# HDaoud/ORBSLAMM

Hardware: AMD Instinct MI355X
Metric: frames/s ORB extract+match, 1241x376 @2000 kp; bit-exact kp/desc vs CPU (higher is better)
Workload: dtype u8

## Files before the change

### include/orbslamm_hip.h

```cpp
#ifndef ORBSLAMM_HIP_H
#define ORBSLAMM_HIP_H

#include <stddef.h>
#include <stdint.h>

#ifdef __cplusplus
extern "C" {
#endif

#define ORBX_MAX_LEVELS 16

enum {
    ORBX_OK = 0,
    ORBX_E_INVALID = -1,
    ORBX_E_NO_DEVICE = -2,
    ORBX_E_HIP = -3,
    ORBX_E_CAPACITY = -4,
    ORBX_E_UNSUPPORTED = -5
};

const char* orbx_last_error(void);
int orbx_device_count(void);
int orbx_device_pci_bus_id(int device, char* out, int cap);
int orbx_device_shader_clock_mhz(int device, float* mhz);
// ... 101 lines not shown
    double ms[ORBX_PROF_MAX];
    int64_t launches[ORBX_PROF_MAX];
} OrbxProfile;
int orbx_set_serial(orbx_t* h, int serial);
int orbx_profile_enable(orbx_t* h, int enable);
int orbx_profile_select(orbx_t* h, const char* kernel);
int orbx_profile_read(orbx_t* h, OrbxProfile* out, int reset);

int orbx_debug_pair_overlap(orbx_t* h, int nb, float target_ms, int* n_kernels, const char** names,
                            float* alone_ms, float* co_ms, int32_t* lds_bytes, int32_t* wg_threads, int32_t* wgs);

int orbx_debug_link_rate(orbx_t* h, size_t up_bytes, size_t down_bytes, int reps, float* h2d_gbs, float* d2h_gbs,
                         float* both_up_gbs, float* both_down_gbs);

int orbx_debug_stage_rows(uint8_t* dst, size_t dpitch, const uint8_t* src, size_t spitch, size_t w, int rows);

typedef struct orbm_handle orbm_t;
int orbm_create(int device, orbm_t** out);
void orbm_destroy(orbm_t* h);
int orbm_thread_handle(int device, orbm_t** out);
int orbm_alloc_stats(orbm_t* h, int64_t* device_allocs, int64_t* host_allocs, int64_t* handles_made);

int orbm_distance_matrix(orbm_t* h, const uint8_t* q, int nq, const uint8_t* t, int nt, int32_t* dist);

int orbm_match_bruteforce(orbm_t* h, const uint8_t* qdesc, const float* qangle, int nq,
                          const uint8_t* tdesc, const float* tangle, int nt,
                          float nnratio, int th_low, int check_ori, int32_t* match, int* nmatches);

typedef struct {
    int32_t n_nodes;
// ... 321 lines not shown
```

### orbslamm_amd/_lib.py

```python
import ctypes as C
import os
import subprocess

import numpy as np

_PKG = os.path.dirname(os.path.abspath(__file__))
_ROOT = os.path.dirname(_PKG)
SO_PATH = os.path.join(_PKG, "liborbslamm_hip.so")
SRC = os.path.join(_PKG, "csrc", "orbslamm_hip.hip")
HIPCC_FLAGS = ["--offload-arch=gfx950", "-O3", "-std=c++17", "-ffp-contract=off", "-fPIC", "-shared"]

ORBX_MAX_LEVELS = 16
ORBX_PROF_MAX = 16
ORBX_OK, ORBX_E_INVALID, ORBX_E_NO_DEVICE, ORBX_E_HIP, ORBX_E_CAPACITY, ORBX_E_UNSUPPORTED = 0, -1, -2, -3, -4, -5

KP_DTYPE = np.dtype([("x", "<f4"), ("y", "<f4"), ("size", "<f4"), ("angle", "<f4"),
                     ("response", "<f4"), ("octave", "<i4"), ("class_id", "<i4")])
assert KP_DTYPE.itemsize == 28


class OrbxParams(C.Structure):
    _fields_ = [("nfeatures", C.c_int32), ("scaleFactor", C.c_float), ("nlevels", C.c_int32),
                ("iniThFAST", C.c_int32), ("minThFAST", C.c_int32)]

# ... 24 lines not shown
    _fields_ = [("minX", C.c_float), ("minY", C.c_float), ("invW", C.c_float), ("invH", C.c_float),
                ("cols", C.c_int32), ("rows", C.c_int32)]


class OrbmProjParams(C.Structure):
    _fields_ = [("mode", C.c_int32), ("nnratio", C.c_float), ("check_ori", C.c_int32), ("th_dist", C.c_int32)]


EXPORTS = [
    "orbx_last_error", "orbx_device_count", "orbx_device_pci_bus_id", "orbx_device_shader_clock_mhz", "orbx_create", "orbx_create_live", "orbx_destroy", "orbx_levels", "orbx_scale_factor",
    "orbx_scale_tables", "orbx_features_per_level", "orbx_umax", "orbx_max_keypoints", "orbx_extract",
    "orbx_extract_batch", "orbx_submit_batch", "orbx_submit_batch_into", "orbx_collect", "orbx_host_alloc", "orbx_collect_view", "orbx_release", "orbx_collect_batch", "orbx_extract_match_batch",
    "orbx_host_alloc_frames", "orbx_host_free", "orbx_host_register", "orbx_host_unregister", "orbx_extract_batch_device", "orbx_device_results", "orbx_download",
    "orbx_pyramid_level", "orbx_compute_stereo_matches", "orbx_level_candidates", "orbx_sync", "orbx_device_alloc", "orbx_device_free", "orbx_upload", "orbx_match_prev_batch_device",
    "orbx_device_matches", "orbx_download_matches", "orbx_reset_stream", "orbx_set_serial", "orbx_profile_enable",
    "orbx_profile_read", "orbx_debug_pair_overlap", "orbx_debug_link_rate", "orbx_debug_stage_rows", "orbx_profile_select", "orbm_create", "orbm_destroy", "orbm_thread_handle", "orbm_alloc_stats", "orbm_distance_matrix", "orbm_match_bruteforce",
    "orbm_search_by_bow", "orbm_search_by_projection", "orbm_search_by_projection_stereo", "orbm_projection_prepare", "orbm_features_in_area", "orbm_window_best",
    "orbm_search_for_initialization", "orbm_search_for_triangulation", "orbm_distinctive_descriptors", "orbm_descriptors_to_text", "orbm_descriptors_from_text", "orbm_undistort_keypoints", "orbm_compute_stereo_from_rgbd", "orbm_frame_create", "orbm_frame_destroy", "orbm_frame_size", "orbm_frame_settle",
    "orbm_frame_download_keys_un", "orbm_search_by_projection_frame", "orbm_frame_compute_bow", "orbm_search_by_bow_frames", "orbm_search_for_initialization_frames", "orbm_window_best_frame", "orbm_search_for_triangulation_frames",
    "orbv_create", "orbv_load_text", "orbv_destroy", "orbv_transform", "orbv_score",
    "orbm_last_search_stats", "orbm_frameset_create", "orbm_frameset_destroy", "orbm_frameset_build", "orbm_frameset_build_from_extractor",
    "orbm_frameset_sync", "orbm_frameset_attach", "orbm_frameset_download", "orbm_track_frames", "orbm_track_local_points", "orbm_track_frame_projected", "orbm_track_results", "orbm_track_stats",
    "orbm_frameset_compute_bow", "orbm_frameset_bow_vector", "orbm_bow_frames", "orbm_bow_results",
]

EXPORTS_KFDB = [
    "orbk_pool_create", "orbk_pool_destroy", "orbk_pool_size", "orbk_pool_set_bow", "orbk_pool_set_bow_from_frameset", "orbk_pool_score",
    "orbk_pool_set_covisibility", "orbk_pool_read_state", "orbk_db_create", "orbk_db_destroy", "orbk_db_add", "orbk_db_erase", "orbk_db_clear",
    "orbk_db_size", "orbk_db_empty", "orbk_db_last_scored", "orbk_detect_relocalization_candidates",
    "orbk_detect_relocalization_candidates_frameset", "orbk_detect_loop_candidates", "orbk_detect_loop_batch",
]
# ... 157 lines not shown
```

### orbslamm_amd/csrc/orbx_geometry.inc

```

static int init_tables(orbx_handle* h)
{
    const OrbxParams& p = h->prm;
    if (p.nlevels < 1 || p.nlevels > ORBX_MAXL || p.nfeatures < 1 || !(p.scaleFactor > 1.0f))
        return fail(ORBX_E_INVALID, "bad ORBextractor parameters");
    const int L = p.nlevels;
    h->nlevels = L;
    const double scaleFactor = (double)p.scaleFactor;
    h->mvScaleFactor[0] = 1.0f;
    h->mvLevelSigma2[0] = 1.0f;
    for (int i = 1; i < L; i++) {
        h->mvScaleFactor[i] = (float)((double)h->mvScaleFactor[i - 1] * scaleFactor);
        h->mvLevelSigma2[i] = h->mvScaleFactor[i] * h->mvScaleFactor[i];
    }
    for (int i = 0; i < L; i++) {
        h->mvInvScaleFactor[i] = 1.0f / h->mvScaleFactor[i];
        h->mvInvLevelSigma2[i] = 1.0f / h->mvLevelSigma2[i];
    }
    const float factor = (float)(1.0 / scaleFactor);
    float nDesired = (float)p.nfeatures * (1 - factor) / (1 - (float)pow((double)factor, (double)L));
    int sum = 0;
    for (int l = 0; l < L - 1; l++) {
        h->mnFeaturesPerLevel[l] = cv_round(nDesired);
        sum += h->mnFeaturesPerLevel[l];
// ... 10 lines not shown
    for (v = kHalfPatch, v0 = 0; v >= vmin; --v) {
        while (h->umax[v0] == h->umax[v0 + 1]) ++v0;
        h->umax[v] = v0;
        ++v0;
    }
    return ORBX_OK;
}

struct HostGeom {
    Geom g;
    std::vector<Cell> cells;
    std::vector<short4> tabs;
    int xoff[ORBX_MAXL], yoff[ORBX_MAXL];
    int tileStrideDw, tileRows, fastListCap, tileRows0, fastListCap0, fastSmapPitch, fastSmapPitch0, nodeCap;
    BlurTiles bt;
    KpBlocks kb;
    int kbTotal;
    std::vector<PyrRange> pyrRanges;
    int pyrBlocks, pyrBufA, pyrBufB, pyrTabCap;
    bool pyrFused;
};

static inline size_t pyr_lds_bytes(int bufA, int bufB, int tabCap) { return ((size_t)bufA + bufB) * 4 + (size_t)tabCap * 16; }

static int build_geometry(const orbx_handle* h, int w, int h0, HostGeom& out)
{
    Geom& g = out.g;
    memset(&g, 0, sizeof g);
    g.nlevels = h->nlevels;
    g.w0 = w; g.h0 = h0;
// ... 117 lines not shown
            auto sat = [](float v) { long r = lrintf(v); return (short)(r > 32767 ? 32767 : (r < -32768 ? -32768 : r)); };
            xt[dx] = make_short4((short)sx, sat((1.f - fx) * 2048), sat(fx * 2048), 0);
        }
        for (int dx = 0; dx < dw; dx++) xt[dx].w = dx < xmax ? 1 : 0;
        out.tabs.insert(out.tabs.end(), xt.begin(), xt.end());
        out.yoff[l] = (int)out.tabs.size();
        for (int dy = 0; dy < dh; dy++) {
            float fy = (float)((dy + 0.5) * scale_y - 0.5);
            int sy = (int)std::floor(fy);
            fy -= sy;
            auto clip = [&](int y) { return y < 0 ? 0 : (y < sh ? y : sh - 1); };
            auto sat = [](float v) { long r = lrintf(v); return (short)(r > 32767 ? 32767 : (r < -32768 ? -32768 : r)); };
            out.tabs.push_back(make_short4((short)clip(sy), (short)clip(sy + 1), sat((1.f - fy) * 2048), sat(fy * 2048)));
        }
    }
    int tb = 0, kb = 0;
    for (int l = 0; l < g.nlevels; l++) {
        out.bt.base[l] = tb;
        out.bt.tilesX[l] = (g.lv[l].w + kBlurTW - 1) / kBlurTW;
        tb += out.bt.tilesX[l] * ((g.lv[l].h + kBlurTH - 1) / kBlurTH);
        out.kb.base[l] = kb;
        kb += (g.lv[l].keptCap + kKpPerBlock - 1) / kKpPerBlock;
    }
    for (int l = g.nlevels; l <= ORBX_MAXL; l++) { out.bt.base[l] = tb; out.kb.base[l] = kb; }
    out.kbTotal = kb;

    out.pyrFused = false;
    const int refine0 = h->maxB <= h->latMaxB ? 1 : 0;
    for (int refine = refine0; refine < 4 && !out.pyrFused; refine++) {
        const int nl = g.nlevels;
        const int top = nl - 1;
        int BX = 4 << refine, BY = 6 << refine;
        while (BX > 1 && g.lv[top].w / BX < 8) BX >>= 1;
        while (BY > 1 && g.lv[top].h / BY < 8) BY >>= 1;
        out.pyrBlocks = BX * BY;
        out.pyrRanges.assign((size_t)out.pyrBlocks * nl, PyrRange{0, 0, 0, 0, 0, 0, 0, 0});
        int maxA = 4, maxB = 4, tabCap = 4;
        for (int bj = 0; bj < BY; bj++)
            for (int bi = 0; bi < BX; bi++) {
// ... 95 lines not shown
```

### orbslamm_amd/csrc/orbx_handle.inc

```

static inline char env_char(const char* name) { const char* e = getenv(name); return e ? e[0] : 0; }
static inline int env_int(const char* name, int unset) { const char* e = getenv(name); return e ? atoi(e) : unset; }

enum ProfId { P_H2D = 0, P_RESIZE, P_FAST, P_DISTRIBUTE, P_BLUR, P_ORIENT_DESC, P_MATCH_BEST2, P_MATCH_ACCEPT, P_MATCH_PRUNE, P_D2H, P_COUNT };
static const char* kProfNames[P_COUNT] = {"h2d", "k_pyramid", "k_fast", "k_distribute", "k_blur",
                                          "k_orient_desc", "k_match_mfma", "k_match_accept", "k_match_prune", "d2h"};
struct ProfSpan { int id; hipEvent_t a, b; };

struct Profiler {
    bool on = false, cur = false;
    int only = -1;
    std::vector<ProfSpan> spans;
    std::vector<hipEvent_t> pool;
    double ms[P_COUNT] = {0};
    int64_t launches[P_COUNT] = {0};
    hipEvent_t get()
    {
        if (!pool.empty()) { hipEvent_t e = pool.back(); pool.pop_back(); return e; }
        hipEvent_t e;
        (void)hipEventCreate(&e);
        return e;
    }
    void begin(int id, hipStream_t s)
    {
// ... 143 lines not shown
struct orbx_handle {
    OrbxParams prm;
    int device = -1;
    int maxW = 0, maxH = 0, maxB = 0;
    int nlevels = 0;
    float mvScaleFactor[ORBX_MAXL], mvInvScaleFactor[ORBX_MAXL], mvLevelSigma2[ORBX_MAXL], mvInvLevelSigma2[ORBX_MAXL];
    int mnFeaturesPerLevel[ORBX_MAXL];
    int umax[16];

    Geom geom;
    int curW = 0, curH = 0;
    std::vector<Cell> cells;
    int tileStrideDw = 0, tileRows = 0, fastListCap = 0, tileRows0 = 0, fastListCap0 = 0, fastSmapPitch = 0, fastSmapPitch0 = 0;
    int nodeCap = 0;
    BlurTiles blurTiles;
    KpBlocks kpBlocks;
    int kpBlocksTotal = 0;
    int pyrBlocks = 0, pyrBufA = 0, pyrBufB = 0, pyrTabCap = 0;
    bool pyrFused = true;
    PyrRange* d_pyrRanges = nullptr; size_t pyrRangesCap = 0;

    hipStream_t stream = nullptr;
    static constexpr int kMaxSplit = 4;
    int nsplit = 2;
    hipStream_t streamP[kMaxSplit] = {nullptr};
    hipEvent_t evStart = nullptr, evPart[kMaxSplit] = {nullptr}, evFast0[kMaxSplit] = {nullptr};
    bool partEverRan[kMaxSplit] = {false};
    int lastParts = 0;
    int prevB = 0, prevSplit = 0;
    hipStream_t stream3 = nullptr;
// ... 85 lines not shown
```

### orbslamm_amd/csrc/orbx_kernels.hip

```cpp
#include <hip/hip_runtime.h>
#include <stdint.h>

#include "orbx_common.hpp"

namespace orbx {

struct FrameSrc {
    const uint8_t* img0;
    int32_t stride0;
    int64_t pitch0;
    uint8_t* pyr;
    uint8_t* blur;
    int32_t f0;
};

__device__ __forceinline__ const uint8_t* level_ptr(const Geom* g, const FrameSrc& s, int f, int l, int& stride)
{
    if (l == 0) { stride = s.stride0; return s.img0 + (int64_t)f * s.pitch0; }
    stride = g->lv[l].stride;
    return s.pyr + (int64_t)f * g->pyrFrameBytes + g->lv[l].pyrOff;
}

__device__ __forceinline__ bool xcd_block_frame(int nframes, int& blk, int& fr)
{
// ... 1136 lines not shown
}

struct BlurTiles { int32_t base[ORBX_MAXL + 1]; int32_t tilesX[ORBX_MAXL]; };

__device__ __forceinline__ int reflect101(int p, int n)
{
    if (n == 1) return 0;
    p = p < 0 ? -p : p;
    p = p >= n ? 2 * n - 2 - p : p;
    while (p < 0 || p >= n) p = p < 0 ? -p : 2 * n - 2 - p;
    return p;
}

constexpr int kBlurTW = 120, kBlurTH = 32;

template <int IN_STRIDE, uint32_t XORV>
__device__ __forceinline__ void blur_load_tile(uint32_t* __restrict__ in, const uint8_t* __restrict__ S, int stride, int w, int h,
                                               int tx0, int ty0, int tid)
{
    constexpr int TW = kBlurTW, TH = kBlurTH;
    constexpr int IN_DW = (TW + 8) / 4;
    bool patchCols = false;
    {
        constexpr int PER = (TH + 6 + 7) / 8;
        const int c = tid & 31, r0 = tid >> 5;
        const int x0 = tx0 - 4 + 4 * c;
        uint32_t regs[PER];
        if (tx0 >= 4 && tx0 + TW + 4 <= w && ty0 >= 3 && ty0 + TH + 3 <= h) {
            const uint8_t* p = S + (int64_t)(ty0 - 3 + r0) * stride + x0;
#pragma unroll
// ... 35 lines not shown
        uint8_t* const inb = (uint8_t*)in;
        if (tx0 == 0 && tid < TH + 6) {
            const uint32_t d1 = in[tid * IN_STRIDE + 1], d2 = in[tid * IN_STRIDE + 2];
            in[tid * IN_STRIDE] = __builtin_amdgcn_perm(d2, d1, 0x01020304u);
        }
        if (tx0 + TW + 4 > w && tid >= 64 && tid < 64 + 4 * (TH + 6)) {
            const int r = (tid - 64) >> 2, k = (tid - 64) & 3;
            const int bd = w + k - (tx0 - 4), bs = w - 2 - k - (tx0 - 4);
            if (bd < 4 * IN_DW && bs >= 0) inb[r * IN_STRIDE * 4 + bd] = inb[r * IN_STRIDE * 4 + bs];
        }
        __syncthreads();
    }
}

struct BlurOps { uint32_t v[4][64][4]; };
constexpr BlurOps make_blur_ops()
{
    constexpr int W[7] = {18, 34, 49, 55, 49, 34, 18};
    BlurOps o{};
    for (int op = 0; op < 4; op++)
        for (int lane = 0; lane < 64; lane++) {
            const int i = lane & 31, hh = lane >> 5;
            for (int b = 0; b < 16; b++) {
                int t = 0;
                if (op < 2) t = (32 * op + 16 * hh + b) - (i + 1);
                else t = (32 * (op - 2) + 8 * (b >> 2) + 4 * hh + (b & 3)) - i;
                const uint32_t val = (t >= 0 && t <= 6) ? (uint32_t)W[t] : 0u;
                o.v[op][lane][b >> 2] |= val << (8 * (b & 3));
            }
        }
    return o;
}
__device__ const BlurOps kBlurOps = make_blur_ops();

constexpr int kBlurMfmaInStride = 36;
constexpr int kBlurMfmaOutStride = 33;
constexpr int kBlurMfmaInWords = (kBlurTH + 6) * kBlurMfmaInStride + 8, kBlurMfmaOutWords = kBlurTH * kBlurMfmaOutStride;

__device__ __forceinline__ void blur_mfma_tile(const Geom* __restrict__ g, const FrameSrc& src, const BlurTiles& bt, const int bx, const int fr,
                                               const bool valid, const int tid, uint32_t* in, uint32_t* outT)
{
    constexpr int TW = kBlurTW, TH = kBlurTH;
    constexpr int IN_STRIDE = kBlurMfmaInStride, OUT_STRIDE = kBlurMfmaOutStride;
    typedef int b4i __attribute__((ext_vector_type(4)));
    typedef int b16i __attribute__((ext_vector_type(16)));
    if (!valid) { __syncthreads(); return; }
    const int f = fr + src.f0;
    int l = 0;
// ... 64 lines not shown
#pragma unroll
    for (int k = 0; k < TH / 8; k++)
        if (rq + 8 * k < nrows) *(uint32_t*)(D + (int64_t)(8 * k) * L.blurStride) = outT[(rq + 8 * k) * OUT_STRIDE + cq];
}

__global__ __launch_bounds__(256, 2) void k_blur_mfma(const Geom* __restrict__ g, FrameSrc src, BlurTiles bt, int nframes)
{
#if ORBX_BLUR_PRIO
    __builtin_amdgcn_s_setprio(ORBX_BLUR_PRIO);
#endif
    __shared__ __attribute__((aligned(16))) uint32_t in[kBlurMfmaInWords];
    __shared__ uint32_t outT[kBlurMfmaOutWords];
    int bx, fr;
    if (!xcd_block_frame(nframes, bx, fr)) return;
    blur_mfma_tile(g, src, bt, bx, fr, true, (int)threadIdx.x, in, outT);
}

__global__ __launch_bounds__(kDistThreads) void k_distribute_blur(DistArgs da, FrameSrc src, BlurTiles bt, int nTiles)
{
    static_assert(kDistThreads == 512, "two blur tiles of 256 threads per block");
    const int nl = da.g->nlevels;
    if ((int)blockIdx.x < nl) { distribute_body<true>(da, (int)blockIdx.x, (int)blockIdx.y); return; }
    __shared__ __attribute__((aligned(16))) uint32_t in2[2][kBlurMfmaInWords];
    __shared__ uint32_t outT2[2][kBlurMfmaOutWords];
    const int half = (int)threadIdx.x >> 8;
    const int tile = 2 * ((int)blockIdx.x - nl) + half;
    blur_mfma_tile(da.g, src, bt, tile, (int)blockIdx.y, tile < nTiles, (int)threadIdx.x & 255, in2[half], outT2[half]);
}

__device__ __forceinline__ void gload_sbase(uint32_t& dst, uint32_t voff, const uint8_t* sbase)
// ... 524 lines not shown
```

### orbslamm_amd/csrc/orbx_pipeline.inc

```

static int configure_shape(orbx_handle* h, int w, int hh)
{
    if (h->curW == w && h->curH == hh) return ORBX_OK;
    if (w > h->maxW || hh > h->maxH) return fail(ORBX_E_INVALID, "frame %dx%d exceeds the handle's maximum %dx%d", w, hh, h->maxW, h->maxH);
    HostGeom hg;
    int rc = build_geometry(h, w, hh, hg);
    if (rc) return rc;
    if (hg.cells.size() > h->cellsCap || hg.tabs.size() > h->tabsCap || (size_t)hg.g.pyrFrameBytes > h->pyrCapFrame ||
        (size_t)hg.g.blurFrameBytes > h->blurCapFrame || (size_t)hg.g.candFrameRecs > h->candCapFrame ||
        (size_t)hg.g.keptFrameRecs > h->keptCapFrame || hg.g.maxKp > h->maxKp)
        return fail(ORBX_E_INVALID, "frame %dx%d needs more scratch than the handle was created with", w, hh);
    const size_t dl = dist_lds_bytes(hg.nodeCap, hg.g.maxCellsPerLevel);
    h->distInLds = dl <= 156 * 1024;
    if (h->distInLds && dl > 48 * 1024 &&
        hipFuncSetAttribute((const void*)k_distribute<true>, hipFuncAttributeMaxDynamicSharedMemorySize, (int)dl) != hipSuccess) {
        (void)hipGetLastError();
        h->distInLds = false;
    }
    if (h->distInLds) {
        h->distBlurOk = hipFuncSetAttribute((const void*)k_distribute_blur, hipFuncAttributeMaxDynamicSharedMemorySize, (int)dl) == hipSuccess;
        if (!h->distBlurOk) (void)hipGetLastError();
    } else {
        const size_t need = dl * (size_t)h->maxB * hg.g.nlevels;
        if (need > h->distScratchBytes && ((rc = sync_all(h)) || (rc = regrow_exact(h->d_distScratch, h->distScratchBytes, need, need)))) return rc;
// ... 8 lines not shown
        if (hg.pyrRanges.size() > h->pyrRangesCap && (rc = regrow_exact(h->d_pyrRanges, h->pyrRangesCap, hg.pyrRanges.size(), hg.pyrRanges.size() * sizeof(PyrRange)))) return rc;
        HIPCHK(hipMemcpy(h->d_pyrRanges, hg.pyrRanges.data(), hg.pyrRanges.size() * sizeof(PyrRange), hipMemcpyHostToDevice));
        h->pyrBlocks = hg.pyrBlocks; h->pyrBufA = hg.pyrBufA; h->pyrBufB = hg.pyrBufB; h->pyrTabCap = hg.pyrTabCap;
        const size_t pl = pyr_lds_bytes(h->pyrBufA, h->pyrBufB, h->pyrTabCap);
        if (pl > 48 * 1024) HIPCHK(hipFuncSetAttribute((const void*)k_pyramid, hipFuncAttributeMaxDynamicSharedMemorySize, (int)pl));
    }
    for (int l = 0; l < ORBX_MAXL; l++) {
        h->tabs.xtab[l] = h->d_tabs + (l < hg.g.nlevels ? hg.xoff[l] : 0);
        h->tabs.ytab[l] = h->d_tabs + (l < hg.g.nlevels ? hg.yoff[l] : 0);
    }
    h->geom = hg.g;
    h->cells = hg.cells;
    h->tileStrideDw = hg.tileStrideDw; h->tileRows = hg.tileRows; h->fastListCap = hg.fastListCap; h->nodeCap = hg.nodeCap;
    h->tileRows0 = hg.tileRows0; h->fastListCap0 = hg.fastListCap0;
    h->fastSmapPitch = hg.fastSmapPitch; h->fastSmapPitch0 = hg.fastSmapPitch0;
    h->blurTiles = hg.bt; h->kpBlocks = hg.kb; h->kpBlocksTotal = hg.kbTotal;
    h->curW = w; h->curH = hh;
    for (int set = 0; set < 2; set++) HIPCHK(hipMemset(r_count(h, set), 0, sizeof(int32_t)));
    return ORBX_OK;
}

static inline unsigned xcd_grid_y(int nb) { return nb < 8 ? (unsigned)nb : 8u * (unsigned)((nb + 7) / 8); }
static inline int xcd_frames(int nb) { return nb >= 8 ? nb : 0; }
template <class T> struct as_declared { using type = T; };

template <class... KArgs>
static int launch_done(orbx_handle* h, int profId, void (*kernel)(KArgs...), dim3 grid, dim3 block, size_t lds, hipStream_t s, hipEvent_t done,
                       typename as_declared<KArgs>::type... args)
{
    h->prof.begin(profId, s);
    if (done && !h->prof.cur) hipExtLaunchKernelGGL(kernel, grid, block, lds, s, nullptr, done, 0, args...);
// ... 56 lines not shown
        }
        if (done) HIPCHK(hipEventRecord(done, s));
        return ORBX_OK;
    }
    bool dist_blur(hipStream_t s) const
    {
        const Geom& g = h->geom;
        if (!h->distInLds || !h->distBlurOk || h->prof.cur || src.f0 != 0) return false;
        const size_t dl = dist_lds_bytes(h->nodeCap, g.maxCellsPerLevel);
        const int nTiles = h->blurTiles.base[g.nlevels];
        DistArgs da{h->d_geom, h->d_candRaw, h->d_candA, h->d_candB, h->d_cells, h->d_cellCount, h->d_candCount, h->d_kept, h->d_keptCount,
                    h->d_errCur, h->nodeCap, src.f0, nullptr, 0, 0};
        hipLaunchKernelGGL(k_distribute_blur, dim3(g.nlevels + (nTiles + 1) / 2, nb), dim3(kDistThreads), dl, s, da, src, h->blurTiles, nTiles);
        return true;
    }
    void blur(hipStream_t s) const
    {
        h->prof.begin(P_BLUR, s);
        hipLaunchKernelGGL(k_blur_mfma, dim3(h->blurTiles.base[h->geom.nlevels], xcd_grid_y(nb)), dim3(256), 0, s, h->d_geom, src, h->blurTiles, nb);
        h->prof.end(s);
    }
    int desc(hipStream_t s, int set, hipEvent_t done = nullptr) const
    {
        if (h->matchPending[set] && h->matchStream[set] != s) HIPCHK(hipStreamWaitEvent(s, h->evMatch[set], 0));
        if (h->evOutOfSet[set] && h->outStream[set] != s) HIPCHK(hipStreamWaitEvent(s, h->evOutOfSet[set], 0));
        for (hipEvent_t e : h->evExtReader[set]) HIPCHK(hipStreamWaitEvent(s, e, 0));
        h->evExtReader[set].clear();
        uint8_t* const xOut = h->fuseExpand ? r_xdesc(h, set) + (size_t)h->xPitch : nullptr;
        return launch_done(h, P_ORIENT_DESC, k_orient_desc, dim3(h->kpBlocksTotal, xcd_grid_y(nb)), dim3(256), 0, s, done, h->d_geom, src, h->kpBlocks, h->d_kept,
                           h->d_keptCount, r_kps(h, set) + h->maxKp, r_desc(h, set) + (size_t)h->maxKp * 32, r_count(h, set) + 1, nb, xOut, h->xPitch, h->xAngOff);
    }
};

struct FrameRange { int f0, f1; };
// ... 39 lines not shown
    }
    h->prevB = B; h->prevSplit = nsplit;
    h->lastParts = 0;
    h->curSet ^= 1;
    const int set = h->curSet;
    const int cellsL0 = g.lv[0].nCells;
    h->lastLat = lat;
    if (lat) {
        hipStream_t sm = h->streamP[0], sa = s0;
        Launcher L{h, src, B};
        if (oneStream) {
            if ((rc = L.pyramid(sm))) return rc;
            L.fast(sm, 0, g.totalCells);
            if (!L.dist_blur(sm)) {
                L.dist(sm, 0, g.nlevels);
                L.blur(sm);
            }
        } else {
            if (evFrames && sIn != sm) HIPCHK(hipStreamWaitEvent(sm, evFrames, 0));
            if (evFrames && sIn != sa) HIPCHK(hipStreamWaitEvent(sa, evFrames, 0));
            if (sIn == sa && h->partEverRan[0]) { if ((rc = flush_part_event(h))) return rc; HIPCHK(hipStreamWaitEvent(sa, h->evPart[0], 0)); }
            L.fast(sa, 0, cellsL0);
            L.dist(sa, 0, 1);
            if ((rc = L.pyramid(sm, h->evPyr[0]))) return rc;
            L.fast(sm, cellsL0, g.totalCells - cellsL0);
            L.dist(sm, 1, g.nlevels - 1);
            HIPCHK(hipStreamWaitEvent(sa, h->evPyr[0], 0));
            L.blur(sa);
            HIPCHK(hipEventRecord(h->evFast0[0], sa));
            HIPCHK(hipStreamWaitEvent(sm, h->evFast0[0], 0));
        }
        if ((rc = L.desc(sm, set, lazyDone ? nullptr : h->evPart[0]))) return rc;
        h->lastParts = 1; h->partLazy = lazyDone; h->partEverRan[0] = true;
    } else {
        for (int part = 0; part < nsplit; part++) {
            const FrameRange fr = part_range(B, part, nsplit);
            const int f0 = fr.f0, nb = fr.f1 - fr.f0;
            if (nb <= 0) continue;
            hipStream_t s = h->serial ? s0 : h->streamP[part];
            hipStream_t s2 = h->serial ? s : s0;
            if (evUploaded) {
                HIPCHK(hipStreamWaitEvent(s, evUploaded[part], 0));
                if (s2 != s) HIPCHK(hipStreamWaitEvent(s2, evUploaded[part], 0));
// ... 1 lines not shown
            if (evFrames && !h->serial) HIPCHK(hipStreamWaitEvent(s, evFrames, 0));
            if (evFrames && !h->serial && sIn != s0 && part == 0) HIPCHK(hipStreamWaitEvent(s0, evFrames, 0));
            src.f0 = f0;
            Launcher L{h, src, nb};
            const bool splitFast = !h->serial && g.nlevels > 1;
            if (splitFast) {
                if (h->partEverRan[part]) HIPCHK(hipStreamWaitEvent(s2, h->evPart[part], 0));
                L.fast(s2, 0, cellsL0);
                HIPCHK(hipEventRecord(h->evFast0[part], s2));
            } else {
                L.fast(s, 0, cellsL0);
            }
            if ((rc = L.pyramid(s))) return rc;
            HIPCHK(hipEventRecord(h->evPyr[part], s));
            HIPCHK(hipStreamWaitEvent(s2, h->evPyr[part], 0));
            L.blur(s2);
            HIPCHK(hipEventRecord(h->evBlur[part], s2));
            L.fast(s, cellsL0, g.totalCells - cellsL0);
            if (splitFast) HIPCHK(hipStreamWaitEvent(s, h->evFast0[part], 0));
            L.dist(s, 0, g.nlevels);
            HIPCHK(hipStreamWaitEvent(s, h->evBlur[part], 0));
            if ((rc = L.desc(s, set))) return rc;
            HIPCHK(hipEventRecord(h->evPart[h->lastParts++], s));
            h->partEverRan[part] = true;
        }
    }
    HIPCHK(hipGetLastError());
    h->lastB = B;
    src.f0 = 0;
    h->lastSrc = src;
    return ORBX_OK;
// ... 87 lines not shown
```

### orbslamm_amd/csrc/orbx_probe.inc

```

extern "C" int orbx_compute_stereo_matches(orbx_t* left, orbx_t* right, int frame, float mb, float mbf,
                                           float* u_right, float* depth, int cap, int* n_left)
{
    int rc = orbx_sync(right);
    if (rc) return rc;
    if ((rc = orbx_sync(left))) return rc;
    if (left->device != right->device) return fail(ORBX_E_INVALID, "the two extractors live on different devices");
    if (left->curW == 0 || left->curW != right->curW || left->curH != right->curH || left->nlevels != right->nlevels)
        return fail(ORBX_E_INVALID, "left and right frames differ in shape or pyramid");
    if (frame < 0 || frame >= left->lastB || frame >= right->lastB) return fail(ORBX_E_INVALID, "frame %d not in the last batches", frame);
    if (!(mb > 0.f) || !(mbf > 0.f)) return fail(ORBX_E_INVALID, "stereo baseline (mb, mbf) must be positive");
    if (left->maxKp >= 65536 || right->maxKp >= 65536) return fail(ORBX_E_UNSUPPORTED, "more than 65535 keypoints per frame");
    int32_t n = 0;
    HIPCHK(hipMemcpy(&n, r_count(left, left->curSet) + 1 + frame, sizeof n, hipMemcpyDeviceToHost));
    if (n_left) *n_left = n;
    if (n > cap) return fail(ORBX_E_CAPACITY, "%d keypoints, caller capacity %d", n, cap);
    if (n == 0) return ORBX_OK;
    const size_t need = (size_t)left->maxKp * 12 + 64;
    if (need > left->stereoBytes && (rc = regrow_exact(left->d_stereo, left->stereoBytes, need, need))) return rc;
    StereoArgs a;
    a.kL = r_kps(left, left->curSet) + (size_t)(frame + 1) * left->maxKp; a.dL = r_desc(left, left->curSet) + (size_t)(frame + 1) * left->maxKp * 32;
    a.nL = r_count(left, left->curSet) + 1 + frame;
    a.kR = r_kps(right, right->curSet) + (size_t)(frame + 1) * right->maxKp; a.dR = r_desc(right, right->curSet) + (size_t)(frame + 1) * right->maxKp * 32;
    a.nR = r_count(right, right->curSet) + 1 + frame;
// ... 142 lines not shown
    HIPCHK_OR(run(false, true, t), cleanup()); if (d2h_gbs) *d2h_gbs = (float)(down_bytes * (double)reps / t / 1e9);
    HIPCHK_OR(run(true, true, t), cleanup());
    if (both_up_gbs) *both_up_gbs = (float)(up_bytes * (double)reps / t / 1e9);
    if (both_down_gbs) *both_down_gbs = (float)(down_bytes * (double)reps / t / 1e9);
    cleanup();
    return ORBX_OK;
}

extern "C" int orbx_debug_stage_rows(uint8_t* dst, size_t dpitch, const uint8_t* src, size_t spitch, size_t w, int rows)
{
    if (!dst || !src || rows < 0 || dpitch < w || spitch < w) return fail(ORBX_E_INVALID, "bad argument");
    stage_rows(dst, dpitch, src, spitch, w, rows);
    return g_stageNt && w >= 128 && !(((uintptr_t)dst | dpitch) & 31) ? 1 : 0;
}

extern "C" int orbx_debug_pair_overlap(orbx_t* h, int nb, float target_ms, int* n_kernels, const char** names,
                                       float* alone_ms, float* co_ms, int32_t* lds_bytes, int32_t* wg_threads, int32_t* wgs)
{
    int rc = orbx_sync(h);
    if (rc) return rc;
    if (h->lastB < 1 || nb < 1 || nb > h->lastB) return fail(ORBX_E_INVALID, "run a batch of at least %d frames first", nb);
    if (!h->streamP[1]) return fail(ORBX_E_UNSUPPORTED, "a latency handle has one chain stream: create the handle with orbx_create and max_batch > 2");
    constexpr int K = 6;
    static const char* kNames[K] = {"k_pyramid", "k_fast", "k_distribute", "k_blur", "k_orient_desc", "k_match_mfma"};
    if (n_kernels) *n_kernels = K;
    const Geom& g = h->geom;
    FrameSrc src = h->lastSrc; src.f0 = 0;
    Launcher L{h, src, nb};
    const int set = h->curSet, cellsL0 = g.lv[0].nCells;
    auto launch = [&](int k, hipStream_t s) {
        switch (k) {
        case 0: (void)L.pyramid(s); break;
        case 1: L.fast(s, 0, cellsL0); L.fast(s, cellsL0, g.totalCells - cellsL0); break;
        case 2: L.dist(s, 0, g.nlevels); break;
        case 3: L.blur(s); break;
        case 4: (void)L.desc(s, set); break;
        default: match_kernels(h, s, set, nb, 0.7f, 50, 1); break;
        }
    };
    if (lds_bytes && wg_threads && wgs) {
        const size_t pl = pyr_lds_bytes(h->pyrBufA, h->pyrBufB, h->pyrTabCap);
        const size_t fl = fast_lds_bytes(h->tileRows, h->tileStrideDw, h->fastSmapPitch, h->fastListCap);
        const int nqb = (h->maxKp + orbm::kMfmaRowsPerBlock - 1) / orbm::kMfmaRowsPerBlock;
        const int32_t l[K] = {(int32_t)pl, (int32_t)fl, (int32_t)(dist_lds_bytes(h->nodeCap, g.maxCellsPerLevel) + 5552), 13464, 31104, orbm::kMfmaLdsBytes};
        const int32_t t[K] = {256, 64, kDistThreads, 256, 256, 256};
        const int32_t w[K] = {h->pyrBlocks * nb, g.totalCells * nb, g.nlevels * nb, h->blurTiles.base[g.nlevels] * nb, h->kpBlocksTotal * nb, nqb * nb};
        for (int k = 0; k < K; k++) { lds_bytes[k] = l[k]; wg_threads[k] = t[k]; wgs[k] = w[k]; }
    }
    for (int k = 0; k < K; k++) if (names) names[k] = kNames[k];
    hipStream_t sa = h->streamP[0], sb = h->streamP[1];
    hipEvent_t e0, e1, eGo;
    HIPCHK(hipEventCreate(&e0)); HIPCHK(hipEventCreate(&e1)); HIPCHK(hipEventCreateWithFlags(&eGo, hipEventDisableTiming));
    auto timed = [&](int i, int j, int ni, int nj, float& ms) -> int {
        HIPCHK(hipEventRecord(eGo, h->stream));
        HIPCHK(hipStreamWaitEvent(sa, eGo, 0));
        if (j >= 0) { HIPCHK(hipStreamWaitEvent(sb, eGo, 0)); for (int r = 0; r < nj / 4; r++) launch(j, sb); }
        HIPCHK(hipEventRecord(e0, sa));
        for (int r = 0; r < ni; r++) { launch(i, sa); if (j >= 0) for (int q = 0; q * ni < nj - nj / 4 && q < 8; q++) launch(j, sb); }
        HIPCHK(hipEventRecord(e1, sa));
        HIPCHK(hipStreamSynchronize(sa)); HIPCHK(hipStreamSynchronize(sb));
        float t = 0; HIPCHK(hipEventElapsedTime(&t, e0, e1));
// ... 23 lines not shown
```

Before: 184,100.

## Add column-walking MFMA blur kernel that reuses vertical halo across row steps

Adds k_blur_walk, in which each workgroup walks down a column strip in runs of 32-row steps. It keeps the previous step's horizontal-blur result in registers so the vertical 7-tap pass does not reload and recompute a halo per tile. The kernel prefetches the next step's rows into registers while the current step computes, and raises its wave priority. Batched throughput paths now use it, while latency paths keep the old tiled kernel. The trade-offs are fewer workgroups, serial dependence along each strip, and a warm-up step per run.

```diff
diff --git a/include/orbslamm_hip.h b/include/orbslamm_hip.h
--- a/include/orbslamm_hip.h
+++ b/include/orbslamm_hip.h
@@ -139,6 +139,8 @@
                          float* both_up_gbs, float* both_down_gbs);
 
 int orbx_debug_stage_rows(uint8_t* dst, size_t dpitch, const uint8_t* src, size_t spitch, size_t w, int rows);
+
+int orbx_debug_blur_ops(int walk, uint32_t* dst, int* steps_per_run);
 
 typedef struct orbm_handle orbm_t;
 int orbm_create(int device, orbm_t** out);
diff --git a/orbslamm_amd/_lib.py b/orbslamm_amd/_lib.py
--- a/orbslamm_amd/_lib.py
+++ b/orbslamm_amd/_lib.py
@@ -62,7 +62,7 @@
     "orbx_host_alloc_frames", "orbx_host_free", "orbx_host_register", "orbx_host_unregister", "orbx_extract_batch_device", "orbx_device_results", "orbx_download",
     "orbx_pyramid_level", "orbx_compute_stereo_matches", "orbx_level_candidates", "orbx_sync", "orbx_device_alloc", "orbx_device_free", "orbx_upload", "orbx_match_prev_batch_device",
     "orbx_device_matches", "orbx_download_matches", "orbx_reset_stream", "orbx_set_serial", "orbx_profile_enable",
-    "orbx_profile_read", "orbx_debug_pair_overlap", "orbx_debug_link_rate", "orbx_debug_stage_rows", "orbx_profile_select", "orbm_create", "orbm_destroy", "orbm_thread_handle", "orbm_alloc_stats", "orbm_distance_matrix", "orbm_match_bruteforce",
+    "orbx_profile_read", "orbx_debug_pair_overlap", "orbx_debug_link_rate", "orbx_debug_stage_rows", "orbx_debug_blur_ops", "orbx_profile_select", "orbm_create", "orbm_destroy", "orbm_thread_handle", "orbm_alloc_stats", "orbm_distance_matrix", "orbm_match_bruteforce",
     "orbm_search_by_bow", "orbm_search_by_projection", "orbm_search_by_projection_stereo", "orbm_projection_prepare", "orbm_features_in_area", "orbm_window_best",
     "orbm_search_for_initialization", "orbm_search_for_triangulation", "orbm_distinctive_descriptors", "orbm_descriptors_to_text", "orbm_descriptors_from_text", "orbm_undistort_keypoints", "orbm_compute_stereo_from_rgbd", "orbm_frame_create", "orbm_frame_destroy", "orbm_frame_size", "orbm_frame_settle",
     "orbm_frame_download_keys_un", "orbm_search_by_projection_frame", "orbm_frame_compute_bow", "orbm_search_by_bow_frames", "orbm_search_for_initialization_frames", "orbm_window_best_frame", "orbm_search_for_triangulation_frames",
diff --git a/orbslamm_amd/csrc/orbx_geometry.inc b/orbslamm_amd/csrc/orbx_geometry.inc
--- a/orbslamm_amd/csrc/orbx_geometry.inc
+++ b/orbslamm_amd/csrc/orbx_geometry.inc
@@ -48,6 +48,7 @@
     int xoff[ORBX_MAXL], yoff[ORBX_MAXL];
     int tileStrideDw, tileRows, fastListCap, tileRows0, fastListCap0, fastSmapPitch, fastSmapPitch0, nodeCap;
     BlurTiles bt;
+    BlurRuns br;
     KpBlocks kb;
     int kbTotal;
     std::vector<PyrRange> pyrRanges;
@@ -195,15 +196,21 @@
             out.tabs.push_back(make_short4((short)clip(sy), (short)clip(sy + 1), sat((1.f - fy) * 2048), sat(fy * 2048)));
         }
     }
-    int tb = 0, kb = 0;
+    int tb = 0, kb = 0, rb = 0;
+    memset(&out.br, 0, sizeof out.br);
     for (int l = 0; l < g.nlevels; l++) {
         out.bt.base[l] = tb;
         out.bt.tilesX[l] = (g.lv[l].w + kBlurTW - 1) / kBlurTW;
         tb += out.bt.tilesX[l] * ((g.lv[l].h + kBlurTH - 1) / kBlurTH);
+        const int steps = blur_walk_steps(g.lv[l].h), nruns = (steps + kBlurRunSteps - 1) / kBlurRunSteps;
+        out.br.base[l] = rb;
+        out.br.colsX[l] = out.bt.tilesX[l];
+        out.br.runSteps[l] = (steps + nruns - 1) / nruns;
+        rb += out.br.colsX[l] * ((steps + out.br.runSteps[l] - 1) / out.br.runSteps[l]);
         out.kb.base[l] = kb;
         kb += (g.lv[l].keptCap + kKpPerBlock - 1) / kKpPerBlock;
     }
-    for (int l = g.nlevels; l <= ORBX_MAXL; l++) { out.bt.base[l] = tb; out.kb.base[l] = kb; }
+    for (int l = g.nlevels; l <= ORBX_MAXL; l++) { out.bt.base[l] = tb; out.br.base[l] = rb; out.kb.base[l] = kb; }
     out.kbTotal = kb;
 
     out.pyrFused = false;
diff --git a/orbslamm_amd/csrc/orbx_handle.inc b/orbslamm_amd/csrc/orbx_handle.inc
--- a/orbslamm_amd/csrc/orbx_handle.inc
+++ b/orbslamm_amd/csrc/orbx_handle.inc
@@ -181,6 +181,7 @@
     int tileStrideDw = 0, tileRows = 0, fastListCap = 0, tileRows0 = 0, fastListCap0 = 0, fastSmapPitch = 0, fastSmapPitch0 = 0;
     int nodeCap = 0;
     BlurTiles blurTiles;
+    BlurRuns blurRuns;
     KpBlocks kpBlocks;
     int kpBlocksTotal = 0;
     int pyrBlocks = 0, pyrBufA = 0, pyrBufB = 0, pyrTabCap = 0;
diff --git a/orbslamm_amd/csrc/orbx_kernels.hip b/orbslamm_amd/csrc/orbx_kernels.hip
--- a/orbslamm_amd/csrc/orbx_kernels.hip
+++ b/orbslamm_amd/csrc/orbx_kernels.hip
@@ -1174,6 +1174,27 @@
 
 constexpr int kBlurTW = 120, kBlurTH = 32;
 
+__device__ __forceinline__ int blur_reflect_row(int yy, int h)
+{
+    return min(max(yy < 0 ? -yy : (yy >= h ? 2 * h - 2 - yy : yy), 0), h - 1);
+}
+
+template <int IN_STRIDE>
+__device__ __forceinline__ void blur_patch_cols(uint32_t* in, int rows, int w, int tx0, int tid, bool left, bool right)
+{
+    constexpr int IN_DW = (kBlurTW + 8) / 4;
+    uint8_t* const inb = (uint8_t*)in;
+    if (left && tid < rows) {
+        const uint32_t d1 = in[tid * IN_STRIDE + 1], d2 = in[tid * IN_STRIDE + 2];
+        in[tid * IN_STRIDE] = __builtin_amdgcn_perm(d2, d1, 0x01020304u);
+    }
+    if (right && tid >= 64 && tid < 64 + 4 * rows) {
+        const int r = (tid - 64) >> 2, k = (tid - 64) & 3;
+        const int bd = w + k - (tx0 - 4), bs = w - 2 - k - (tx0 - 4);
+        if (bd < 4 * IN_DW && bs >= 0) inb[r * IN_STRIDE * 4 + bd] = inb[r * IN_STRIDE * 4 + bs];
+    }
+}
+
 template <int IN_STRIDE, uint32_t XORV>
 __device__ __forceinline__ void blur_load_tile(uint32_t* __restrict__ in, const uint8_t* __restrict__ S, int stride, int w, int h,
                                                int tx0, int ty0, int tid)
@@ -1239,7 +1260,7 @@
 }
 
 struct BlurOps { uint32_t v[4][64][4]; };
-constexpr BlurOps make_blur_ops()
+constexpr BlurOps make_blur_ops(bool walk)
 {
     constexpr int W[7] = {18, 34, 49, 55, 49, 34, 18};
     BlurOps o{};
@@ -1249,6 +1270,7 @@
             for (int b = 0; b < 16; b++) {
                 int t = 0;
                 if (op < 2) t = (32 * op + 16 * hh + b) - (i + 1);
+                else if (walk) t = (8 * (b >> 2) + 4 * hh + (b & 3)) - i + (op == 2 ? -26 : 6);
                 else t = (32 * (op - 2) + 8 * (b >> 2) + 4 * hh + (b & 3)) - i;
                 const uint32_t val = (t >= 0 && t <= 6) ? (uint32_t)W[t] : 0u;
                 o.v[op][lane][b >> 2] |= val << (8 * (b & 3));
@@ -1256,7 +1278,7 @@
         }
     return o;
 }
-__device__ const BlurOps kBlurOps = make_blur_ops();
+__device__ const BlurOps kBlurOps = make_blur_ops(false), kBlurWalkOps = make_blur_ops(true);
 
 constexpr int kBlurMfmaInStride = 36;
 constexpr int kBlurMfmaOutStride = 33;
@@ -1351,6 +1373,150 @@
     int bx, fr;
     if (!xcd_block_frame(nframes, bx, fr)) return;
     blur_mfma_tile(g, src, bt, bx, fr, true, (int)threadIdx.x, in, outT);
+}
+
+#ifndef ORBX_BLUR_RUN
+#define ORBX_BLUR_RUN 12
+#endif
+#ifndef ORBX_BLUR_WALK_PRIO
+#define ORBX_BLUR_WALK_PRIO 2
+#endif
+constexpr int kBlurRunSteps = ORBX_BLUR_RUN;
+struct BlurRuns { int32_t base[ORBX_MAXL + 1]; int32_t colsX[ORBX_MAXL]; int32_t runSteps[ORBX_MAXL]; };
+__host__ __device__ constexpr int blur_walk_steps(int h) { return (h + 37) / 32; }
+constexpr int kBlurWalkInWords = kBlurTH * kBlurMfmaInStride + 8;
+
+__global__ __launch_bounds__(256, 2) void k_blur_walk(const Geom* __restrict__ g, FrameSrc src, BlurRuns br, int nframes)
+{
+#if ORBX_BLUR_WALK_PRIO
+    __builtin_amdgcn_s_setprio(ORBX_BLUR_WALK_PRIO);
+#endif
+    constexpr int TW = kBlurTW, TH = kBlurTH;
+    constexpr int IN_STRIDE = kBlurMfmaInStride, OUT_STRIDE = kBlurMfmaOutStride;
+    typedef int b4i __attribute__((ext_vector_type(4)));
+    typedef int b16i __attribute__((ext_vector_type(16)));
+    __shared__ __attribute__((aligned(16))) uint32_t in[kBlurWalkInWords];
+    __shared__ uint32_t outT[kBlurMfmaOutWords];
+    int bx, fr;
+    if (!xcd_block_frame(nframes, bx, fr)) return;
+    const int tid = (int)threadIdx.x;
+    const int f = fr + src.f0;
+    int l = 0;
+    while (l + 1 < g->nlevels && bx >= br.base[l + 1]) l++;
+    const int rIdx = bx - br.base[l];
+    const int run = rIdx / br.colsX[l];
+    const int tx0 = (rIdx - run * br.colsX[l]) * TW;
+    const LevelGeom& L = g->lv[l];
+    const int w = L.w, h = L.h;
+    const int tBeg = run * br.runSteps[l], tEnd = min(blur_walk_steps(h), tBeg + br.runSteps[l]);
+    int stride;
+    const uint8_t* S = level_ptr(g, src, f, l, stride);
+    const int wave = tid >> 6, lane = tid & 63, hh = lane >> 5, m = lane & 31;
+    const b4i* ops = (const b4i*)kBlurWalkOps.v;
+    const b4i hB0 = ops[lane], hB1 = ops[64 + lane], vAp = ops[128 + lane], vAc = ops[192 + lane];
+    const int c = tid & 31, r0 = tid >> 5;
+    const int x0 = tx0 - 4 + 4 * c;
+    const bool colIn = tx0 >= 4 && tx0 + TW + 4 <= w;
+    const bool big = w >= 12 && h >= 12;
+    const bool patchL = big && tx0 == 0, patchR = big && tx0 + TW + 4 > w;
+    const bool edge = !(x0 >= 0 && x0 + 3 < w);
+    const int xs = min(max(x0, 0), (w - 1) & ~3);
+    auto ld = [&](uint32_t off) { return *(const uint32_t*)(S + off); };
+    uint32_t regs[TH / 8] = {0, 0, 0, 0};
+    auto fetch = [&](int tt, bool warm) {
+        const int y0 = 32 * tt - 3 + r0;
+        if (colIn && tt > 0 && 32 * tt + 29 <= h) {
+#pragma unroll
+            for (int k = 0; k < TH / 8; k++)
+                if (!warm || k == TH / 8 - 1) regs[k] = ld((uint32_t)(y0 * stride + xs) + (uint32_t)(8 * k * stride));
+        } else if (big) {
+#pragma unroll
+            for (int k = 0; k < TH / 8; k++) {
+                const int yy = y0 + 8 * k;
+                if (!warm || k == TH / 8 - 1) regs[k] = ld((uint32_t)(blur_reflect_row(yy, h) * stride + xs));
+            }
+        } else {
+#pragma unroll
+            for (int k = 0; k < TH / 8; k++) {
+                const uint8_t* row = S + (uint32_t)(reflect101(y0 + 8 * k, h) * stride);
+                uint32_t v = *(const uint32_t*)(row + xs);
+                if (edge) {
+                    v = 0;
+#pragma unroll
+                    for (int b = 0; b < 4; b++) v |= (uint32_t)row[reflect101(x0 + b, w)] << (8 * b);
+                }
+                regs[k] = v;
+            }
+        }
+    };
+    const bool active = tx0 + 32 * wave < w;
+    const uint8_t* const inb = (const uint8_t*)in + 32 * wave + 16 * hh + m * (IN_STRIDE * 4);
+    uint8_t* const ob = (uint8_t*)outT + (4 * hh) * (OUT_STRIDE * 4) + 32 * wave + m;
+    const int cq = tid & 31, rq = tid >> 5;
+    const bool stores = cq < TW / 4 && tx0 + 4 * cq < w;
+    uint8_t* const D = src.blur + (int64_t)f * g->blurFrameBytes + L.blurOff;
+    const int xq = tx0 + 4 * cq;
+    const int bstride = L.blurStride;
+    b16i c128, cLo;
+#pragma unroll
+    for (int r = 0; r < 16; r++) { c128[r] = 128; cLo[r] = 257 * 32896 + 32768; }
+    asm volatile("" : "+v"(c128), "+v"(cLo));
+    const b16i zero = {0, 0, 0, 0, 0, 0, 0, 0, 0, 0, 0, 0, 0, 0, 0, 0};
+    b4i loP = {0, 0, 0, 0}, hiP = {0, 0, 0, 0};
+
+    int t = tBeg > 0 ? tBeg - 1 : 0;
+    fetch(t, tBeg > 0);
+    for (; t < tEnd; t++) {
+        const bool warm = t < tBeg;
+#pragma unroll
+        for (int k = 0; k < TH / 8; k++) in[(r0 + 8 * k) * IN_STRIDE + c] = regs[k] ^ 0x80808080u;
+        __syncthreads();
+        if (patchL || patchR) {
+            blur_patch_cols<IN_STRIDE>(in, TH, w, tx0, tid, patchL, patchR);
+            __syncthreads();
+        }
+        if (t + 1 < tEnd) fetch(t + 1, false);
+        if (active) {
+            const b4i a0 = *(const b4i*)inb, a1 = *(const b4i*)(inb + 32);
+            b16i G = __builtin_amdgcn_mfma_i32_32x32x32_i8(a0, hB0, c128, 0, 0, 0);
+            G = __builtin_amdgcn_mfma_i32_32x32x32_i8(a1, hB1, G, 0, 0, 0);
+            b4i loC, hiC;
+#pragma unroll
+            for (int gq = 0; gq < 4; gq++) {
+                const uint32_t t0 = __builtin_amdgcn_perm((uint32_t)G[4 * gq + 1], (uint32_t)G[4 * gq], 0x05010400u);
+                const uint32_t t1 = __builtin_amdgcn_perm((uint32_t)G[4 * gq + 3], (uint32_t)G[4 * gq + 2], 0x05010400u);
+                loC[gq] = (int)(__builtin_amdgcn_perm(t1, t0, 0x05040100u) ^ 0x80808080u);
+                hiC[gq] = (int)__builtin_amdgcn_perm(t1, t0, 0x07060302u);
+            }
+            if (!warm) {
+                b16i aHi = __builtin_amdgcn_mfma_i32_32x32x32_i8(vAp, hiP, zero, 0, 0, 0);
+                aHi = __builtin_amdgcn_mfma_i32_32x32x32_i8(vAc, hiC, aHi, 0, 0, 0);
+                b16i aLo = __builtin_amdgcn_mfma_i32_32x32x32_i8(vAp, loP, cLo, 0, 0, 0);
+                aLo = __builtin_amdgcn_mfma_i32_32x32x32_i8(vAc, loC, aLo, 0, 0, 0);
+#pragma unroll
+                for (int r = 0; r < 16; r++) {
+                    const uint32_t v = min((uint32_t)((aHi[r] << 8) + aLo[r]), 0xFFFFFFu);
+                    ob[((r & 3) + 8 * (r >> 2)) * (OUT_STRIDE * 4)] = (uint8_t)(v >> 16);
+                }
+            }
+            loP = loC; hiP = hiC;
+        }
+        __syncthreads();
+        if (!warm && stores) {
+            const int yb = 32 * t - 6 + rq;
+            if (t > 0 && 32 * t + 26 <= h) {
+#pragma unroll
+                for (int k = 0; k < TH / 8; k++)
+                    *(uint32_t*)(D + ((uint32_t)(yb * bstride + xq) + (uint32_t)(8 * k * bstride))) = outT[(rq + 8 * k) * OUT_STRIDE + cq];
+            } else {
+#pragma unroll
+                for (int k = 0; k < TH / 8; k++) {
+                    const int y = yb + 8 * k;
+                    if (y >= 0 && y < h) *(uint32_t*)(D + (uint32_t)(y * bstride + xq)) = outT[(rq + 8 * k) * OUT_STRIDE + cq];
+                }
+            }
+        }
+    }
 }
 
 __global__ __launch_bounds__(kDistThreads) void k_distribute_blur(DistArgs da, FrameSrc src, BlurTiles bt, int nTiles)
diff --git a/orbslamm_amd/csrc/orbx_pipeline.inc b/orbslamm_amd/csrc/orbx_pipeline.inc
--- a/orbslamm_amd/csrc/orbx_pipeline.inc
+++ b/orbslamm_amd/csrc/orbx_pipeline.inc
@@ -46,7 +46,7 @@
     h->tileStrideDw = hg.tileStrideDw; h->tileRows = hg.tileRows; h->fastListCap = hg.fastListCap; h->nodeCap = hg.nodeCap;
     h->tileRows0 = hg.tileRows0; h->fastListCap0 = hg.fastListCap0;
     h->fastSmapPitch = hg.fastSmapPitch; h->fastSmapPitch0 = hg.fastSmapPitch0;
-    h->blurTiles = hg.bt; h->kpBlocks = hg.kb; h->kpBlocksTotal = hg.kbTotal;
+    h->blurTiles = hg.bt; h->blurRuns = hg.br; h->kpBlocks = hg.kb; h->kpBlocksTotal = hg.kbTotal;
     h->curW = w; h->curH = hh;
     for (int set = 0; set < 2; set++) HIPCHK(hipMemset(r_count(h, set), 0, sizeof(int32_t)));
     return ORBX_OK;
@@ -133,10 +133,11 @@
         hipLaunchKernelGGL(k_distribute_blur, dim3(g.nlevels + (nTiles + 1) / 2, nb), dim3(kDistThreads), dl, s, da, src, h->blurTiles, nTiles);
         return true;
     }
-    void blur(hipStream_t s) const
+    void blur(hipStream_t s, bool lat = false) const
     {
         h->prof.begin(P_BLUR, s);
-        hipLaunchKernelGGL(k_blur_mfma, dim3(h->blurTiles.base[h->geom.nlevels], xcd_grid_y(nb)), dim3(256), 0, s, h->d_geom, src, h->blurTiles, nb);
+        if (lat) hipLaunchKernelGGL(k_blur_mfma, dim3(h->blurTiles.base[h->geom.nlevels], xcd_grid_y(nb)), dim3(256), 0, s, h->d_geom, src, h->blurTiles, nb);
+        else hipLaunchKernelGGL(k_blur_walk, dim3(h->blurRuns.base[h->geom.nlevels], xcd_grid_y(nb)), dim3(256), 0, s, h->d_geom, src, h->blurRuns, nb);
         h->prof.end(s);
     }
     int desc(hipStream_t s, int set, hipEvent_t done = nullptr) const
@@ -206,7 +207,7 @@
             L.fast(sm, 0, g.totalCells);
             if (!L.dist_blur(sm)) {
                 L.dist(sm, 0, g.nlevels);
-                L.blur(sm);
+                L.blur(sm, true);
             }
         } else {
             if (evFrames && sIn != sm) HIPCHK(hipStreamWaitEvent(sm, evFrames, 0));
@@ -218,7 +219,7 @@
             L.fast(sm, cellsL0, g.totalCells - cellsL0);
             L.dist(sm, 1, g.nlevels - 1);
             HIPCHK(hipStreamWaitEvent(sa, h->evPyr[0], 0));
-            L.blur(sa);
+            L.blur(sa, true);
             HIPCHK(hipEventRecord(h->evFast0[0], sa));
             HIPCHK(hipStreamWaitEvent(sm, h->evFast0[0], 0));
         }
@@ -250,7 +251,7 @@
             if ((rc = L.pyramid(s))) return rc;
             HIPCHK(hipEventRecord(h->evPyr[part], s));
             HIPCHK(hipStreamWaitEvent(s2, h->evPyr[part], 0));
-            L.blur(s2);
+            L.blur(s2, B <= h->latMaxB);
             HIPCHK(hipEventRecord(h->evBlur[part], s2));
             L.fast(s, cellsL0, g.totalCells - cellsL0);
             if (splitFast) HIPCHK(hipStreamWaitEvent(s, h->evFast0[part], 0));
diff --git a/orbslamm_amd/csrc/orbx_probe.inc b/orbslamm_amd/csrc/orbx_probe.inc
--- a/orbslamm_amd/csrc/orbx_probe.inc
+++ b/orbslamm_amd/csrc/orbx_probe.inc
@@ -180,6 +180,15 @@
     return g_stageNt && w >= 128 && !(((uintptr_t)dst | dpitch) & 31) ? 1 : 0;
 }
 
+extern "C" int orbx_debug_blur_ops(int walk, uint32_t* dst, int* steps_per_run)
+{
+    if (!dst) return fail(ORBX_E_INVALID, "bad argument");
+    static constexpr BlurOps kTile = make_blur_ops(false), kWalk = make_blur_ops(true);
+    memcpy(dst, walk ? kWalk.v : kTile.v, sizeof kTile.v);
+    if (steps_per_run) *steps_per_run = kBlurRunSteps;
+    return ORBX_OK;
+}
+
 extern "C" int orbx_debug_pair_overlap(orbx_t* h, int nb, float target_ms, int* n_kernels, const char** names,
                                        float* alone_ms, float* co_ms, int32_t* lds_bytes, int32_t* wg_threads, int32_t* wgs)
 {
@@ -208,9 +217,9 @@
         const size_t pl = pyr_lds_bytes(h->pyrBufA, h->pyrBufB, h->pyrTabCap);
         const size_t fl = fast_lds_bytes(h->tileRows, h->tileStrideDw, h->fastSmapPitch, h->fastListCap);
         const int nqb = (h->maxKp + orbm::kMfmaRowsPerBlock - 1) / orbm::kMfmaRowsPerBlock;
-        const int32_t l[K] = {(int32_t)pl, (int32_t)fl, (int32_t)(dist_lds_bytes(h->nodeCap, g.maxCellsPerLevel) + 5552), 13464, 31104, orbm::kMfmaLdsBytes};
+        const int32_t l[K] = {(int32_t)pl, (int32_t)fl, (int32_t)(dist_lds_bytes(h->nodeCap, g.maxCellsPerLevel) + 5552), (kBlurWalkInWords + kBlurMfmaOutWords) * 4, 31104, orbm::kMfmaLdsBytes};
         const int32_t t[K] = {256, 64, kDistThreads, 256, 256, 256};
-        const int32_t w[K] = {h->pyrBlocks * nb, g.totalCells * nb, g.nlevels * nb, h->blurTiles.base[g.nlevels] * nb, h->kpBlocksTotal * nb, nqb * nb};
+        const int32_t w[K] = {h->pyrBlocks * nb, g.totalCells * nb, g.nlevels * nb, h->blurRuns.base[g.nlevels] * nb, h->kpBlocksTotal * nb, nqb * nb};
         for (int k = 0; k < K; k++) { lds_bytes[k] = l[k]; wg_threads[k] = t[k]; wgs[k] = w[k]; }
     }
     for (int k = 0; k < K; k++) if (names) names[k] = kNames[k];
```

After: 188,600, median of 6. +2.4%, better.
